# DassHydro-dev/smash

Hardware: AMD Instinct MI355X
Metric: cell-timesteps/s, forward+adjoint sweep (higher is better)
Workload: dtype f32

## Files before the change

### smash_amd/csrc/sx_kernels.h

```cpp
#pragma once

#include <hip/hip_runtime.h>

#include <climits>

#include "sx_ops.h"
#include "sx_tangent.h"
#include "sx_vic.h"

#define SX_BT 4
#define SX_VBLOCK 256

__device__ __forceinline__ void sx_lds_barrier() {
    __builtin_amdgcn_fence(__ATOMIC_RELEASE, "workgroup", "local");
    __builtin_amdgcn_s_barrier();
    __builtin_amdgcn_fence(__ATOMIC_ACQUIRE, "workgroup", "local");
}

__device__ __forceinline__ void sx_lds_wave_fence() {
    __builtin_amdgcn_fence(__ATOMIC_RELEASE, "workgroup", "local");
    __builtin_amdgcn_wave_barrier();
    __builtin_amdgcn_fence(__ATOMIC_ACQUIRE, "workgroup", "local");
}

typedef float sx_f4v __attribute__((ext_vector_type(4)));
__device__ __forceinline__ float4 sx_gload4(const float4* p) {
#if defined(__HIP_DEVICE_COMPILE__)
    const sx_f4v v = *(const __attribute__((address_space(1))) sx_f4v*)p;
    return make_float4(v.x, v.y, v.z, v.w);
#else
    return *p;
#endif
}
#ifndef SX_R_NT
#define SX_R_NT 0
#endif
__device__ __forceinline__ float4 sx_gload4s(const float4* p) {
#if defined(__HIP_DEVICE_COMPILE__)
    if (SX_R_NT & 1) {
        const sx_f4v v = __builtin_nontemporal_load((const __attribute__((address_space(1))) sx_f4v*)p);
        return make_float4(v.x, v.y, v.z, v.w);
    }
#endif
    return sx_gload4(p);
}
__device__ __forceinline__ void sx_gstore4s(float4* p, const float4& q) {
#if defined(__HIP_DEVICE_COMPILE__)
    if (SX_R_NT & 2) {
        sx_f4v v; v.x = q.x; v.y = q.y; v.z = q.z; v.w = q.w;
        __builtin_nontemporal_store(v, (__attribute__((address_space(1))) sx_f4v*)p);
        return;
    }
    {
        sx_f4v v; v.x = q.x; v.y = q.y; v.z = q.z; v.w = q.w;
        *(__attribute__((address_space(1))) sx_f4v*)p = v;
        return;
    }
#endif
    *p = q;
}
__device__ __forceinline__ void sx_gstore4(float4* p, const float4& q) {
#if defined(__HIP_DEVICE_COMPILE__)
    sx_f4v v; v.x = q.x; v.y = q.y; v.z = q.z; v.w = q.w;
    *(__attribute__((address_space(1))) sx_f4v*)p = v;
#else
    *p = q;
#endif
}
__device__ __forceinline__ float sx_gload1(const float* p) {
#if defined(__HIP_DEVICE_COMPILE__)
    return *(const __attribute__((address_space(1))) float*)p;
#else
    return *p;
#endif
}

__device__ __forceinline__ void sx_pin(float4& v) {
    asm volatile("" : "+v"(v.x), "+v"(v.y), "+v"(v.z), "+v"(v.w) : : "memory");
}

__device__ __forceinline__ void sx_pin1(float& v) { asm volatile("" : "+v"(v) : : "memory"); }
__device__ __forceinline__ void sx_pinu(unsigned& v) { asm volatile("" : "+v"(v) : : "memory"); }

typedef __attribute__((address_space(1))) int sx_gint;
#define SX_PROG_STALL(A) ((A).prog + (A).ngroups)
#define SX_PROG_TICKET(A) ((A).prog + (A).ngroups + 1)
#define SX_PROG_EXTRA 8
#ifndef SX_PK
#define SX_PK 16
#endif
#define SX_SPIN_LIMIT (1 << 22)
__device__ __forceinline__ void sx_wait_prog(const int* prog, int need, int& seen, int* stalled, int limit, int tag = -1) {
    if (seen >= need) return;
    int spins = 0;
    while (seen < need) {
        seen = __hip_atomic_load((const sx_gint*)prog, __ATOMIC_RELAXED, __HIP_MEMORY_SCOPE_AGENT);
        if (seen < need) {
            const bool out = ++spins > limit;
            if (out || (spins & 1023) == 0) {
                if (out) {
                    if (atomicCAS(stalled + 3, 0, tag + 2) == 0) { stalled[4] = (int)(prog - stalled); stalled[5] = need; stalled[6] = seen; }
                    __hip_atomic_store((sx_gint*)stalled, 1, __ATOMIC_RELAXED, __HIP_MEMORY_SCOPE_AGENT);
                }
                if (out || __hip_atomic_load((const sx_gint*)stalled, __ATOMIC_RELAXED, __HIP_MEMORY_SCOPE_AGENT)) { seen = 0x7fffffff; break; }
            }
            __builtin_amdgcn_s_sleep(32);
        }
    }
    __builtin_amdgcn_fence(__ATOMIC_ACQUIRE, "agent");
}
__device__ __forceinline__ void sx_publish(int* prog, int blocks) {
    __builtin_amdgcn_fence(__ATOMIC_RELEASE, "agent");
    __hip_atomic_store((sx_gint*)prog, blocks, __ATOMIC_RELAXED, __HIP_MEMORY_SCOPE_AGENT);
}

struct SxDeviceArrays {
    int n, npad, nt, Tc;
    int k0, k1;
    int nx;
    float dt, dx;
    const float* prcp; const float* pet;
    const unsigned short* prcp16; const float* petd; const float* pet_ratio;
    float prcp_c, prcp_gap; int hour0;
    float *ci, *cp, *cft, *cst, *exc, *lr;
    float* px[3]; float* px_b[3];
    float *rt_a, *rt_f, *rt_denf, *rt_denb;
    int* flwacc;
    float *hi, *hp, *hft, *hst, *hlr;
    float *ci_b, *cp_b, *cft_b, *cst_b, *exc_b, *lr_b, *hi_b, *hp_b, *hft_b, *hst_b, *hlr_b;
    float *qtT, *hrT;
    int hr_skew;
    float *qtdT, *xdT, *qgd;
    float* qdT;
    float *tape_hi, *tape_hp, *tape_hft, *tape_hst;
    float* ckpt_hi;
    float* xT;
    float* qsk; int cs0, ncs;
    float *qg, *qgb;
    int* cell_gauge;
    const int *g_slot_begin, *g_dmax;
    const int *s_cell, *s_stage, *s_sub, *s_wsub, *s_child, *s_ccount, *s_parent, *s_xout;
    const int *x_prod, *x_cons;
    int* prog;
    int ngroups;
    int spin_limit;
    int mute_group;
    long long* gtime;
};

struct SxStageTables {
    const int* wb_slot0; const int* wb_n; const int* wb_smin; const int* wb_spread;
    const int* fifo_g; const int* fifo_s;
};
#ifndef SX_STG_PF
#define SX_STG_PF 16
#endif
#ifndef SX_STG_WAVES
// ... 257 lines not shown
        sx_row_store4<SX_NT>(A.qtT + (size_t)tq * npad * 4, kb * 4u, q[0], q[1], q[2], q[3]);
    }
    A.hi[k] = husl1; A.hp[k] = husl2; A.hft[k] = hlsl;
}

#ifndef SX_VADJ_WAVES_VIC
#define SX_VADJ_WAVES_VIC 3
#endif
template <bool CF>
__global__ __launch_bounds__(SX_VBLOCK, SX_VADJ_WAVES_VIC) void sx_k_vert_adj_vic(SxDeviceArrays A, int t0, int T) {
    SX_LIBM_INIT();
    const int k = A.k0 + blockIdx.x * SX_VBLOCK + threadIdx.x;
    if (k >= A.k1) return;
    const size_t npad = (size_t)A.npad;
    const SxVicParams P = sx_vic_load(A, k);
    float cusl2_m4, cusl2_m5;
    sx_pow_m4_m5(P.cusl2, &cusl2_m4, &cusl2_m5);
    SxVicGrads G;
    G.b_b = A.ci_b[k]; G.cusl1_b = A.cp_b[k]; G.cusl2_b = A.cft_b[k]; G.clsl_b = A.cst_b[k]; G.ks_b = A.exc_b[k];
    G.ds_b = A.px_b[0][k]; G.dsm_b = A.px_b[1][k]; G.ws_b = A.px_b[2][k];
    G.husl1_b = A.hi_b[k]; G.husl2_b = A.hp_b[k]; G.hlsl_b = A.hft_b[k];
    const unsigned kb = (unsigned)k * 4u;
    SxForcing<CF> F(A, kb, t0 + T - 1);
    float n_h1 = 0.f, n_h2 = 0.f, n_hl = 0.f, n_q = 0.f;
    auto fetch = [&](int tt, bool first) {
        const size_t o = (size_t)tt * npad;
        F.template request<SX_VADJ_NT, true>(t0 + tt, first);
        n_h1 = sx_row_load<SX_VADJ_NT>(A.tape_hi + o, kb); n_h2 = sx_row_load<SX_VADJ_NT>(A.tape_hp + o, kb);
        n_hl = sx_row_load<SX_VADJ_NT>(A.tape_hft + o, kb);
        n_q = sx_row_load(A.qtT + (size_t)(tt >> 2) * npad * 4 + (tt & 3), kb * 4u);
    };
    if (T > 0) fetch(T - 1, true);
    for (int tt = T - 1; tt >= 0; --tt) {
        float h1 = n_h1, h2 = n_h2, hl = n_hl, q_b = n_q;
        F.hold();
        sx_pin1(h1); sx_pin1(h2); sx_pin1(hl); sx_pin1(q_b);
        if (tt > 0) fetch(tt - 1, false);
        sx_vic_step_b(P, cusl2_m4, cusl2_m5, F.prcp(), F.pet(), h1, h2, hl, q_b, G);
    }
    A.ci_b[k] = G.b_b; A.cp_b[k] = G.cusl1_b; A.cft_b[k] = G.cusl2_b; A.cst_b[k] = G.clsl_b; A.exc_b[k] = G.ks_b;
    A.px_b[0][k] = G.ds_b; A.px_b[1][k] = G.dsm_b; A.px_b[2][k] = G.ws_b;
    A.hi_b[k] = G.husl1_b; A.hp_b[k] = G.husl2_b; A.hft_b[k] = G.hlsl_b;
}

__global__ __launch_bounds__(SX_VBLOCK) void sx_k_vert_fwd_vic_d(SxDeviceArrays A, int t0, int T) {
    SX_LIBM_INIT();
    const int k = A.k0 + blockIdx.x * SX_VBLOCK + threadIdx.x;
    if (k >= A.k1) return;
    const size_t npad = (size_t)A.npad;
    const SxVicParams P = sx_vic_load(A, k);
    SxVicTan D;
    D.b_d = A.ci_b[k]; D.cusl1_d = A.cp_b[k]; D.cusl2_d = A.cft_b[k]; D.clsl_d = A.cst_b[k]; D.ks_d = A.exc_b[k];
    D.ds_d = A.px_b[0][k]; D.dsm_d = A.px_b[1][k]; D.ws_d = A.px_b[2][k];
    float cusl2_m4, cusl2_m5;
    sx_pow_m4_m5(P.cusl2, &cusl2_m4, &cusl2_m5);
    SxVD husl1 = sx_vd(A.hi[k], A.hi_b[k]), husl2 = sx_vd(A.hp[k], A.hp_b[k]), hlsl = sx_vd(A.hft[k], A.hft_b[k]);
    float* qt = A.qtT + (size_t)k * 4;
    float* qd = A.qtdT + (size_t)k * 4;
    for (int tt = 0; tt < T; ++tt) {
        float prcp, pet;
        sx_forcing_at(A, t0 + tt, (unsigned)k * 4u, prcp, pet);
        const SxVD r = sx_vic_step_d(P, D, cusl2_m4, cusl2_m5, prcp, pet, husl1, husl2, hlsl);
        const size_t o = (size_t)(tt >> 2) * npad * 4 + (tt & 3);
        qt[o] = r.v; qd[o] = r.d;
    }
    A.hi[k] = husl1.v; A.hi_b[k] = husl1.d; A.hp[k] = husl2.v; A.hp_b[k] = husl2.d; A.hft[k] = hlsl.v; A.hft_b[k] = hlsl.d;
}

template <int ST>
__global__ __launch_bounds__(SX_VBLOCK) void sx_k_vert_fwd_d(SxDeviceArrays A, int t0, int T) {
    SX_LIBM_INIT();
    const int k = A.k0 + blockIdx.x * SX_VBLOCK + threadIdx.x;
    if (k >= A.k1) return;
    const size_t npad = (size_t)A.npad;
    SxCellParams P;
    P.ci = (ST == 2 || ST == 3) ? A.ci[k] : 1.f;
    P.cp = A.cp[k];
    P.cft = A.cft[k];
    P.cst = (ST == 3) ? A.cst[k] : 1.f;
    P.exc = (ST != 4) ? A.exc[k] : 0.f;
    sx_cell_params_init(P);
    SxAdjParams Q;
    Q.cst_m5 = 1.f;
    sx_pow_m4_m5(P.cft, &P.cft_m4, &Q.cft_m5);
    P.cst_m4 = 1.f;
    if (ST == 3) sx_pow_m4_m5(P.cst, &P.cst_m4, &Q.cst_m5);
    Q.dcft2 = sx_mkdiv(P.cft * P.cft);
    Q.dcst2 = sx_mkdiv(P.cst * P.cst);
    Q.dcp2 = sx_mkdiv(P.cp * P.cp);
    SxTanParams D;
    D.ci_d = (ST == 2 || ST == 3) ? A.ci_b[k] : 0.f;
    D.cp_d = A.cp_b[k];
    D.cft_d = A.cft_b[k];
    D.cst_d = (ST == 3) ? A.cst_b[k] : 0.f;
    D.exc_d = (ST != 4) ? A.exc_b[k] : 0.f;
    SxDual hi = sx_mk(0.f, 0.f), hp, hft, hst = sx_mk(0.f, 0.f);
    if (ST == 2 || ST == 3) hi = sx_mk(A.hi[k], A.hi_b[k]);
    hp = sx_mk(A.hp[k], A.hp_b[k]);
    hft = sx_mk(A.hft[k], A.hft_b[k]);
    if (ST == 3) hst = sx_mk(A.hst[k], A.hst_b[k]);
    float4* qt4 = reinterpret_cast<float4*>(A.qtT) + k;
    float4* qd4 = reinterpret_cast<float4*>(A.qtdT) + k;
    for (int tq = 0; tq * 4 < T; ++tq) {
        float q[4] = {0.f, 0.f, 0.f, 0.f}, qd[4] = {0.f, 0.f, 0.f, 0.f};
#pragma unroll
        for (int i = 0; i < 4; ++i) {
            const int tt = tq * 4 + i;
            if (tt < T) {
                float prcp, pet;
                sx_forcing_at(A, t0 + tt, (unsigned)k * 4u, prcp, pet);
                const SxDual r = sx_vertical_step_d<ST>(P, Q, D, prcp, pet, hi, hp, hft, hst);
                q[i] = r.v; qd[i] = r.d;
            }
        }
        qt4[(size_t)tq * npad] = make_float4(q[0], q[1], q[2], q[3]);
        qd4[(size_t)tq * npad] = make_float4(qd[0], qd[1], qd[2], qd[3]);
    }
    if (ST == 2 || ST == 3) { A.hi[k] = hi.v; A.hi_b[k] = hi.d; }
    A.hp[k] = hp.v; A.hp_b[k] = hp.d;
    A.hft[k] = hft.v; A.hft_b[k] = hft.d;
    if (ST == 3) { A.hst[k] = hst.v; A.hst_b[k] = hst.d; }
}

#ifndef SX_MU
#define SX_MU 4
#endif
#ifndef SX_MU_F
#define SX_MU_F SX_MU
#endif
#ifndef SX_MU_A
#define SX_MU_A SX_MU
#endif
#ifndef SX_MAXGROUP
#define SX_MAXGROUP 512
#endif
#ifndef SX_R_PRIO
#define SX_R_PRIO 0
#endif
#ifndef SX_RLB_F
#define SX_RLB_F 1
#endif
#ifndef SX_RLB_A
#define SX_RLB_A 1
#endif

__device__ __forceinline__ int sx_next_ticket(const SxDeviceArrays& A) {
    __shared__ int s_ticket;
    __builtin_amdgcn_s_barrier();
    if (threadIdx.x == 0) s_ticket = __hip_atomic_fetch_add((sx_gint*)SX_PROG_TICKET(A), 1, __ATOMIC_RELAXED, __HIP_MEMORY_SCOPE_AGENT);
    __syncthreads();
    return s_ticket;
}

template <bool TAPE, bool CHAIN, int TMODE>
__device__ __forceinline__ void sx_route_fwd_group(const SxDeviceArrays& A, const int g, const int g0, const int gend, const int t0, const int T) {
    constexpr bool TAN = (TMODE == 2);
    constexpr int MU = SX_MU_F, PK = SX_PK * 4 / MU;
    constexpr bool DFORM = (TMODE == 1);
    extern __shared__ __attribute__((aligned(16))) float4 sx_lds[];
    const int sb = A.g_slot_begin[g], m = A.g_slot_begin[g + 1] - sb, dmax = A.g_dmax[g];
    const int j = threadIdx.x, M = blockDim.x;
    bool valid = j < m;
    const int nb = (T + SX_BT - 1) / SX_BT;
    if (A.gtime && j == 0) A.gtime[2 * g] = wall_clock64();

    int cell = -1, stage = 0, sub = 0, ccount = 0, xout = -1, xin = -1, gid = -1;
    unsigned ch01 = ~0u, ch23 = ~0u, ch45 = ~0u, ch67 = ~0u;
    float a = 0.f, f = 0.f, den = 1.f, hlr = 0.f, ad = 0.f;
    bool hasup = false;
    const int nsubw = __builtin_amdgcn_readfirstlane(m > 0 ? A.s_wsub[sb + min(j, m - 1)] : 1);
    if (valid && A.s_cell[sb + j] == INT_MIN) valid = false;
    if (valid) {
        const int c = A.s_cell[sb + j];
        stage = A.s_stage[sb + j];
        sub = A.s_sub[sb + j];
        if (c >= 0) {
            cell = c;
            const int4 cw = reinterpret_cast<const int4*>(A.s_child)[sb + j];
            ch01 = (unsigned)cw.x; ch23 = (unsigned)cw.y; ch45 = (unsigned)cw.z; ch67 = (unsigned)cw.w;
            ccount = A.s_ccount[sb + j]; xout = A.s_xout[sb + j];
            a = A.rt_a[c]; f = A.rt_f[c]; den = (TAN || DFORM) ? A.rt_denb[c] : A.rt_denf[c]; hlr = TAN ? A.hlr_b[c] : A.hlr[c];
            if (TAN) { const float lrv = A.lr[c]; ad = a * ((A.dt / (60.f * lrv)) * A.lr_b[c] / lrv); }
            hasup = A.flwacc[c] > 1;
            gid = A.cell_gauge[c];
        } else {
            xin = -1 - c;
        }
    }
    const float dt = A.dt, dx = A.dx;
    const SxDiv dden = sx_mkdiv(den), ddt = sx_mkdiv(dt);
    const int* wprog = nullptr;
    int seen = 0;
    if (CHAIN && xin >= 0) { const int pg = A.x_prod[xin]; if (pg >= g0 && pg < gend) wprog = A.prog + pg; }
    const bool staged = CHAIN && !TAN && A.qsk != nullptr && valid && !wprog;
    const float4* src = staged ? reinterpret_cast<const float4*>(A.qsk) + (size_t)stage * A.ncs + (sb + j - A.cs0)
                      : (cell >= 0) ? reinterpret_cast<const float4*>(TAN ? A.qtdT : A.qtT) + cell
                                    : reinterpret_cast<const float4*>(TAN ? A.xdT : A.xT) + (xin >= 0 ? xin : 0);
    const size_t sstride = staged ? (size_t)A.ncs : (cell >= 0) ? (size_t)A.npad : (size_t)A.nx;
    float4* x4 = reinterpret_cast<float4*>(TAN ? A.xdT : A.xT);
    float4* hr4 = reinterpret_cast<float4*>(A.hrT);
    const int hs = A.hr_skew ? stage : 0;
    float* gauge_out = TAN ? A.qgd : A.qg;
    const float4 zero4 = make_float4(0.f, 0.f, 0.f, 0.f);
    auto fetch = [&](int tb) -> float4 { return cell >= 0 ? sx_gload4s(src + (size_t)tb * sstride) : sx_gload4(src + (size_t)tb * sstride); };

    float4 nxt[MU], outq[MU], outh[MU], nhr[MU];
    if (CHAIN && wprog) sx_wait_prog(wprog, min(MU - stage, nb), seen, SX_PROG_STALL(A), A.spin_limit, g);
#pragma unroll
    for (int u = 0; u < MU; ++u) {
        const int tb = u - stage;
        nxt[u] = (valid && tb >= 0 && tb < nb) ? fetch(tb) : zero4;
        nhr[u] = (TAN && valid && cell >= 0 && tb >= 0 && tb < nb) ? sx_gload4(hr4 + (size_t)(tb + hs) * A.npad + cell) : zero4;
        outq[u] = zero4; outh[u] = zero4;
    }
    const int nsuper = nb + dmax;
    const int nmacro = (nsuper + MU - 1) / MU;
    for (int mw = 0; mw <= nmacro; ++mw) {
        float4 cur[MU], chr[MU];
#pragma unroll
        for (int u = 0; u < MU; ++u) { cur[u] = nxt[u]; sx_pin(cur[u]); if (TAN) { chr[u] = nhr[u]; sx_pin(chr[u]); } }
        if (CHAIN) asm volatile("s_waitcnt vmcnt(0)" ::: "memory");
        if (mw > 0 && cell >= 0) {
#pragma unroll
            for (int u = 0; u < MU; ++u) {
                const int tb = MU * (mw - 1) + u - stage;
                if (tb >= 0 && tb < nb) {
                    if (xout >= 0) x4[(size_t)tb * A.nx + xout] = outq[u];
                    if (TAPE) sx_gstore4s(hr4 + (size_t)(tb + hs) * A.npad + cell, outh[u]);
                    if (A.qdT) reinterpret_cast<float4*>(A.qdT)[(size_t)tb * A.npad + cell] = outq[u];
                    if (gid >= 0) {
                        const float qv[4] = {outq[u].x, outq[u].y, outq[u].z, outq[u].w};
#pragma unroll
                        for (int i = 0; i < SX_BT; ++i)
                            if (tb * SX_BT + i < T) gauge_out[(size_t)gid * A.nt + t0 + tb * SX_BT + i] = qv[i];
                    }
                }
            }
        }
        if (mw == nmacro) break;
        if (CHAIN && wprog) sx_wait_prog(wprog, min(MU * (mw + 2) - stage, nb), seen, SX_PROG_STALL(A), A.spin_limit, g);
#pragma unroll
        for (int u = 0; u < MU; ++u) {
            const int tb = MU * (mw + 1) + u - stage;
            nxt[u] = (valid && tb >= 0 && tb < nb) ? fetch(tb) : zero4;
            if (TAN) nhr[u] = (valid && cell >= 0 && tb >= 0 && tb < nb) ? sx_gload4(hr4 + (size_t)(tb + hs) * A.npad + cell) : zero4;
        }
#pragma unroll
        for (int u = 0; u < MU; ++u) {
            const int w = MU * mw + u;
            const int tb = w - stage;
            const bool act = valid && tb >= 0 && tb < nb;
            float4* pub = sx_lds + (size_t)(w & 1) * M;
            auto child_val = [&](unsigned e) -> float4 {
                const float4* row = sx_lds + (size_t)((w + 1 + (int)((e >> 15) & 1u)) & 1) * M;
                return row[min((int)(e & 0x7fffu), M - 1)];
            };
          auto sub_pass = [&](const int sl) {
            if (act && sub == sl) {
                const int tl = tb * SX_BT;
                if (cell >= 0) {
                    float s[SX_BT];
                    {
                        const float4 v0 = child_val(ch01 & 0xffffu), v1 = child_val(ch01 >> 16);
                        const bool h0 = ccount > 0, h1 = ccount > 1;
                        s[0] = (h0 ? v0.x : 0.f) + (h1 ? v1.x : 0.f); s[1] = (h0 ? v0.y : 0.f) + (h1 ? v1.y : 0.f);
                        s[2] = (h0 ? v0.z : 0.f) + (h1 ? v1.z : 0.f); s[3] = (h0 ? v0.w : 0.f) + (h1 ? v1.w : 0.f);
                    }
                    for (int c = 2; c < ccount; ++c) {
                        const unsigned wd = c < 4 ? ch23 : c < 6 ? ch45 : ch67;
                        const float4 v = child_val((wd >> ((c & 1) * 16)) & 0xffffu);
                        s[0] = s[0] + v.x; s[1] = s[1] + v.y; s[2] = s[2] + v.z; s[3] = s[3] + v.w;
                    }
                    const float qt[SX_BT] = {cur[u].x, cur[u].y, cur[u].z, cur[u].w};
                    float q[SX_BT], hr[SX_BT], qup[SX_BT], qro[SX_BT];
                    {
                        float nq[SX_BT], dq[SX_BT];
#pragma unroll
                        for (int i = 0; i < SX_BT; ++i) nq[i] = DFORM ? s[i] : s[i] * dt;
                        sx_div4(dq, nq, dden);
#pragma unroll
                        for (int i = 0; i < SX_BT; ++i) qup[i] = hasup ? (DFORM ? dt * dq[i] : dq[i]) : 0.f;
                    }
                    if (!TAN) {
#pragma unroll
                        for (int i = 0; i < SX_BT; ++i) {
                            const bool live = tl + i < T;
                            const float hr_imd = hlr + qup[i];
                            const float hnew = hr_imd * a;
                            qro[i] = hr_imd - hnew;
                            hr[i] = live ? hr_imd : 0.f;
                            hlr = live ? hnew : hlr;
                        }
                        float nq[SX_BT], dq[SX_BT];
#pragma unroll
                        for (int i = 0; i < SX_BT; ++i) nq[i] = DFORM ? qt[i] + f * qro[i] : (qt[i] + qro[i] * f) * dx * dx * 0.001f;
                        sx_div4(dq, nq, ddt);
#pragma unroll
                        for (int i = 0; i < SX_BT; ++i) {
                            const float v = DFORM ? (0.001f * (dx * dx)) * dq[i] : dq[i];
                            q[i] = (tl + i < T) ? v : 0.f;
                        }
                    } else {
                        const float hrv[SX_BT] = {chr[u].x, chr[u].y, chr[u].z, chr[u].w};
#pragma unroll
                        for (int i = 0; i < SX_BT; ++i) {
                            const bool live = tl + i < T;
                            const float hr_imd_d = hlr + qup[i];
                            const float hnew_d = a * hr_imd_d + hrv[i] * ad;
                            qro[i] = hr_imd_d - hnew_d;
                            hr[i] = 0.f;
                            hlr = live ? hnew_d : hlr;
                        }
#pragma unroll
                        for (int i = 0; i < SX_BT; ++i) {
                            const float v = sx_div((0.001f * (dx * dx)) * (qt[i] + f * qro[i]), ddt);
                            q[i] = (tl + i < T) ? v : 0.f;
                        }
                    }
                    const float4 q4 = make_float4(q[0], q[1], q[2], q[3]);
                    pub[j] = q4;
                    outq[u] = q4;
                    outh[u] = make_float4(hr[0], hr[1], hr[2], hr[3]);
                } else {
                    pub[j] = cur[u];
                }
            }
          };
            if (nsubw == 1) sub_pass(0);
            else for (int sl = 0; sl < nsubw; ++sl) { sub_pass(sl); if (sl + 1 < nsubw) sx_lds_wave_fence(); }
            sx_lds_barrier();
            if (CHAIN && u == 0 && j == 0 && mw % PK == 0) { const int done = min(MU * (mw - 1) - dmax, nb); if (done > 0 && g != A.mute_group) sx_publish(A.prog + g, done); }
        }
    }
    if (valid && cell >= 0) { if (TAN) A.hlr_b[cell] = hlr; else A.hlr[cell] = hlr; }
    if (A.gtime && j == 0) A.gtime[2 * g + 1] = wall_clock64();
    if (CHAIN) {
        asm volatile("s_waitcnt vmcnt(0)" ::: "memory");
        __builtin_amdgcn_s_barrier();
        if (j == 0 && g != A.mute_group) sx_publish(A.prog + g, nb);
    }
}

template <bool TAPE, bool CHAIN, int TMODE = 0>
__global__ __launch_bounds__(SX_MAXGROUP, SX_RLB_F) void sx_k_route_fwd(SxDeviceArrays A, int g0, int gend, int t0, int T) {
    if (SX_R_PRIO) __builtin_amdgcn_s_setprio(SX_R_PRIO);
    if (!CHAIN) { sx_route_fwd_group<TAPE, false, TMODE>(A, g0 + (int)blockIdx.x, g0, gend, t0, T); return; }
    for (;;) {
        const int ticket = sx_next_ticket(A);
        if (ticket >= gend - g0) break;
        sx_route_fwd_group<TAPE, CHAIN, TMODE>(A, g0 + ticket, g0, gend, t0, T);
    }
}

template <bool CHAIN>
__device__ __forceinline__ void sx_route_adj_group(const SxDeviceArrays& A, const int g, const int g0, const int gend, const int t0, const int T) {
    constexpr int MU = SX_MU_A, PK = SX_PK * 4 / MU;
    extern __shared__ __attribute__((aligned(16))) float4 sx_lds[];
    const int sb = A.g_slot_begin[g], m = A.g_slot_begin[g + 1] - sb, dmax = A.g_dmax[g];
    const int j = threadIdx.x, M = blockDim.x;
    bool valid = j < m;
    const int nb = (T + SX_BT - 1) / SX_BT;
    if (A.gtime && j == 0) A.gtime[2 * (A.ngroups + g)] = wall_clock64();

    int cell = -1, rstage = 0, sub = 0, par = -1, xout = -1, xin = -1, gid = -1;
    bool psame = false;
    float a = 0.f, f = 0.f, den = 1.f, lr = 1.f, hr_b = 0.f, lr_b = 0.f;
    bool hasup = false;
    const int nsubw = __builtin_amdgcn_readfirstlane(m > 0 ? A.s_wsub[sb + min(j, m - 1)] : 1);
    if (valid && A.s_cell[sb + j] == INT_MIN) valid = false;
    if (valid) {
        const int c = A.s_cell[sb + j];
        rstage = dmax - A.s_stage[sb + j];
        sub = A.s_sub[sb + j];
        par = A.s_parent[sb + j];
        if (par >= 0) { psame = (par & 0x40000000) != 0; par &= 0xffff; }
        if (c >= 0) {
            cell = c;
            xout = A.s_xout[sb + j];
            a = A.rt_a[c]; f = A.rt_f[c]; den = A.rt_denb[c]; lr = A.lr[c];
            hr_b = A.hlr_b[c]; lr_b = A.lr_b[c];
            hasup = A.flwacc[c] > 1;
            gid = A.cell_gauge[c];
        } else {
            xin = -1 - c;
        }
    }
    const float dt = A.dt, dx = A.dx;
    const SxDiv dden = sx_mkdiv(den), ddt = sx_mkdiv(dt), dlr = sx_mkdiv((lr * lr) * 60.f);
    float4* x4 = reinterpret_cast<float4*>(A.xT);
    const float4* hr4p = reinterpret_cast<const float4*>(A.hrT);
    const int hs = A.hr_skew ? dmax - rstage : 0;
    float4* qt4 = reinterpret_cast<float4*>(A.qtT);
    const float4 zero4 = make_float4(0.f, 0.f, 0.f, 0.f);
    const bool root_in = (cell >= 0 && par < 0 && xout >= 0);
    const bool staged = CHAIN && A.qsk != nullptr && valid && (cell >= 0 || (xin >= 0 && !(A.x_prod[xin] >= g0 && A.x_prod[xin] < gend)));
    float4* const dst = staged ? reinterpret_cast<float4*>(A.qsk) + (size_t)(dmax - rstage) * A.ncs + (sb + j - A.cs0)
                               : (cell >= 0) ? qt4 + cell : x4 + (xin >= 0 ? xin : 0);
    const size_t dstride = staged ? (size_t)A.ncs : (cell >= 0) ? (size_t)A.npad : (size_t)A.nx;

    const float* seedp = (gid >= 0) ? A.qgb + (size_t)gid * A.nt + t0 : nullptr;
    auto load_seed = [&](int tb) -> float4 {
        float4 v = make_float4(0.f, 0.f, 0.f, 0.f);
        if (gid >= 0) {
            const int tl = tb * SX_BT;
            if (tl + 0 < T) v.x = sx_gload1(seedp + tl + 0);
            if (tl + 1 < T) v.y = sx_gload1(seedp + tl + 1);
            if (tl + 2 < T) v.z = sx_gload1(seedp + tl + 2);
            if (tl + 3 < T) v.w = sx_gload1(seedp + tl + 3);
        }
        return v;
    };
    const int* wprog = nullptr;
    int seen = 0;
    if (CHAIN && root_in) { const int cg = A.x_cons[xout]; if (cg >= g0 && cg < gend) wprog = A.prog + cg; }
    auto fetch_in = [&](int tb) -> float4 { return sx_gload4(x4 + (size_t)tb * A.nx + xout); };
    float4 nhr[MU], nin[MU], nsd[MU], outq[MU];
    if (CHAIN && wprog) sx_wait_prog(wprog, min(MU - rstage, nb), seen, SX_PROG_STALL(A), A.spin_limit, g);
#pragma unroll
    for (int u = 0; u < MU; ++u) {
        const int tbr = u - rstage;
        const int tb = nb - 1 - tbr;
        const bool ok = valid && tbr >= 0 && tbr < nb;
        nhr[u] = (ok && cell >= 0) ? sx_gload4s(hr4p + (size_t)(tb + hs) * A.npad + cell) : zero4;
        nin[u] = (ok && root_in) ? fetch_in(tb) : zero4;
        nsd[u] = ok ? load_seed(tb) : zero4;
        outq[u] = zero4;
    }
    const int nsuper = nb + dmax;
    const int nmacro = (nsuper + MU - 1) / MU;
    for (int mw = 0; mw <= nmacro; ++mw) {
        float4 chr[MU], cin[MU], csd[MU];
#pragma unroll
        for (int u = 0; u < MU; ++u) {
            chr[u] = nhr[u]; cin[u] = nin[u]; csd[u] = nsd[u];
            sx_pin(chr[u]); sx_pin(cin[u]); sx_pin(csd[u]);
        }
        if (CHAIN) asm volatile("s_waitcnt vmcnt(0)" ::: "memory");
        if (mw > 0 && valid) {
#pragma unroll
            for (int u = 0; u < MU; ++u) {
                const int tbr = MU * (mw - 1) + u - rstage;
                if (tbr >= 0 && tbr < nb) {
                    const int tb = nb - 1 - tbr;
                    sx_gstore4(dst + (size_t)tb * dstride, outq[u]);
                }
            }
        }
        if (mw == nmacro) break;
        if (CHAIN && wprog) sx_wait_prog(wprog, min(MU * (mw + 2) - rstage, nb), seen, SX_PROG_STALL(A), A.spin_limit, g);
#pragma unroll
        for (int u = 0; u < MU; ++u) {
            const int tbr = MU * (mw + 1) + u - rstage;
            const int tb = nb - 1 - tbr;
            const bool ok = valid && tbr >= 0 && tbr < nb;
            nhr[u] = (ok && cell >= 0) ? sx_gload4s(hr4p + (size_t)(tb + hs) * A.npad + cell) : zero4;
            nin[u] = (ok && root_in) ? fetch_in(tb) : zero4;
            nsd[u] = ok ? load_seed(tb) : zero4;
        }
#pragma unroll
        for (int u = 0; u < MU; ++u) {
            const int w = MU * mw + u;
            const int tbr = w - rstage;
            const bool act = valid && tbr >= 0 && tbr < nb;
            float4* pub = sx_lds + (size_t)(w & 1) * M;
            const float4* prev = sx_lds + (size_t)((w + 1) & 1) * M;
          auto sub_pass = [&](const int sl) {
            if (act && sub == sl) {
                const int tb = nb - 1 - tbr;
                const int tl = tb * SX_BT;
                float4 in4 = cin[u];
                if (par >= 0) in4 = psame ? pub[par] : prev[par];
                if (cell >= 0) {
                    const float hrv[SX_BT] = {chr[u].x, chr[u].y, chr[u].z, chr[u].w};
                    const float inv[SX_BT] = {in4.x, in4.y, in4.z, in4.w};
                    const float sdv[SX_BT] = {csd[u].x, csd[u].y, csd[u].z, csd[u].w};
                    float pb[SX_BT], qtb[SX_BT];
                    float tmpb[SX_BT], qrb[SX_BT], himb[SX_BT], a1b[SX_BT];
                    float nq[SX_BT];
#pragma unroll
                    for (int i = SX_BT - 1; i >= 0; --i) {
                        float q_b = 0.f;
                        if (gid >= 0) q_b = q_b + sdv[i];
                        q_b = q_b + inv[i];
                        nq[i] = (dx * dx) * 0.001f * q_b;
                    }
                    sx_div4(tmpb, nq, ddt);
#pragma unroll
                    for (int i = SX_BT - 1; i >= 0; --i) qrb[i] = f * tmpb[i];
#pragma unroll
                    for (int i = SX_BT - 1; i >= 0; --i) {
                        const bool live = tl + i < T;
                        const float hb1 = hr_b - qrb[i];
                        himb[i] = qrb[i] + a * hb1;
                        a1b[i] = a * hrv[i] * hb1;
                        hr_b = live ? himb[i] : hr_b;
                    }
                    float na[SX_BT], nh[SX_BT], da[SX_BT], dh[SX_BT];
#pragma unroll
                    for (int i = 0; i < SX_BT; ++i) { na[i] = dt * a1b[i]; nh[i] = dt * himb[i]; }
                    sx_div4(da, na, dlr);
                    sx_div4(dh, nh, dden);
#pragma unroll
                    for (int i = SX_BT - 1; i >= 0; --i) {
                        const bool live = tl + i < T;
                        const float lnew = lr_b + da[i];
                        lr_b = live ? lnew : lr_b;
                        pb[i] = (live && hasup) ? dh[i] : 0.f;
                        qtb[i] = live ? tmpb[i] : 0.f;
                    }
                    pub[j] = make_float4(pb[0], pb[1], pb[2], pb[3]);
                    outq[u] = make_float4(qtb[0], qtb[1], qtb[2], qtb[3]);
                } else {
                    outq[u] = in4;
                }
            }
          };
            if (nsubw == 1) sub_pass(0);
            else for (int sl = nsubw - 1; sl >= 0; --sl) { sub_pass(sl); if (sl > 0) sx_lds_wave_fence(); }
            sx_lds_barrier();
            if (CHAIN && u == 0 && j == 0 && mw % PK == 0) { const int done = min(MU * (mw - 1) - dmax, nb); if (done > 0 && g != A.mute_group) sx_publish(A.prog + g, done); }
        }
    }
    if (valid && cell >= 0) { A.hlr_b[cell] = hr_b; A.lr_b[cell] = lr_b; }
    if (A.gtime && j == 0) A.gtime[2 * (A.ngroups + g) + 1] = wall_clock64();
    if (CHAIN) {
        asm volatile("s_waitcnt vmcnt(0)" ::: "memory");
        __builtin_amdgcn_s_barrier();
        if (j == 0 && g != A.mute_group) sx_publish(A.prog + g, nb);
    }
}

template <bool CHAIN>
__global__ __launch_bounds__(SX_MAXGROUP, SX_RLB_A) void sx_k_route_adj(SxDeviceArrays A, int g0, int gend, int t0, int T) {
    if (SX_R_PRIO) __builtin_amdgcn_s_setprio(SX_R_PRIO);
    if (!CHAIN) { sx_route_adj_group<false>(A, g0 + (int)blockIdx.x, g0, gend, t0, T); return; }
    for (;;) {
        const int ticket = sx_next_ticket(A);
        if (ticket >= gend - g0) break;
        sx_route_adj_group<CHAIN>(A, gend - 1 - ticket, g0, gend, t0, T);
    }
}

#ifndef SX_VADJ_WAVES
#define SX_VADJ_WAVES 5
#endif
template <int ST, bool CF>
#ifndef SX_VADJ_WAVES_GRC
#if SX_EXACT_LIBM
#define SX_VADJ_WAVES_GRC 1
#else
#define SX_VADJ_WAVES_GRC 5
#endif
#endif
__global__ __launch_bounds__(SX_VBLOCK, (ST == 2 && CF) ? SX_VADJ_WAVES : (ST == 3 && CF) ? SX_VADJ_WAVES_GRC : 1)
void sx_k_vert_adj(SxDeviceArrays A, int t0, int T) {
    SX_LIBM_INIT();
    const int k = A.k0 + blockIdx.x * SX_VBLOCK + threadIdx.x;
    if (k >= A.k1) return;
    const size_t npad = (size_t)A.npad;
    SxCellParams P;
    P.ci = (ST == 2 || ST == 3) ? A.ci[k] : 1.f;
    P.cp = A.cp[k];
    P.cft = A.cft[k];
    P.cst = (ST == 3) ? A.cst[k] : 1.f;
    P.exc = (ST != 4) ? A.exc[k] : 0.f;
    sx_cell_params_init(P);
    SxAdjParams Q;
    Q.cst_m5 = 1.f;
    sx_pow_m4_m5(P.cft, &P.cft_m4, &Q.cft_m5);
    P.cst_m4 = 1.f;
    if (ST == 3) sx_pow_m4_m5(P.cst, &P.cst_m4, &Q.cst_m5);
    Q.dcft2 = sx_mkdiv(P.cft * P.cft);
    Q.dcst2 = sx_mkdiv(P.cst * P.cst);
    Q.dcp2 = sx_mkdiv(P.cp * P.cp);
    SxCellGrads G;
    G.ci_b = (ST == 2 || ST == 3) ? A.ci_b[k] : 0.f;
    G.cp_b = A.cp_b[k];
    G.cft_b = A.cft_b[k];
    G.cst_b = (ST == 3) ? A.cst_b[k] : 0.f;
    G.exc_b = (ST != 4) ? A.exc_b[k] : 0.f;
    G.hi_b = (ST == 2 || ST == 3) ? A.hi_b[k] : 0.f;
    G.hp_b = A.hp_b[k];
    G.hft_b = A.hft_b[k];
    G.hst_b = (ST == 3) ? A.hst_b[k] : 0.f;
    const unsigned kb = (unsigned)k * 4u;
    SxForcing<CF> F(A, kb, t0 + T - 1);
    float n_hi = 0.f, n_hp = 0.f, n_hft = 0.f, n_hst = 0.f, n_q = 0.f;
    const bool hi_taped = (ST == 2 || ST == 3) && A.tape_hi != nullptr;
    const size_t olast = (size_t)(T > 0 ? T - 1 : 0) * npad;
    const float* r_hi = hi_taped ? A.tape_hi + olast : nullptr;
    const float* r_hp = A.tape_hp + olast;
    const float* r_hft = A.tape_hft + olast;
    const float* r_hst = (ST == 3) ? A.tape_hst + olast : nullptr;
    auto fetch = [&](int tt, bool first) {
        F.template request<SX_VADJ_NT, true>(t0 + tt, first);
        if (hi_taped) { n_hi = sx_row_load<SX_VADJ_NT>(r_hi, kb); r_hi -= npad; }
        n_hp = sx_row_load<SX_VADJ_NT>(r_hp, kb); n_hft = sx_row_load<SX_VADJ_NT>(r_hft, kb);
        r_hp -= npad; r_hft -= npad;
        if (ST == 3) { n_hst = sx_row_load<SX_VADJ_NT>(r_hst, kb); r_hst -= npad; }
        n_q = sx_row_load(A.qtT + (size_t)(tt >> 2) * npad * 4 + (tt & 3), kb * 4u);
    };
    __shared__ float s_hi[(ST == 2 || ST == 3) ? SX_HIK : 1][SX_VBLOCK];
    if (T > 0) fetch(T - 1, true);
    for (int tb = (T - 1) / SX_HIK; tb >= 0; --tb) {
        const int tt0 = tb * SX_HIK, len = min(SX_HIK, T - tt0);
        if ((ST == 2 || ST == 3) && !hi_taped) {
            float fp[SX_HIK], fe[SX_HIK];
#pragma unroll
            for (int j = 0; j < SX_HIK; ++j) sx_forcing_at(A, t0 + tt0 + (j < len ? j : 0), kb, fp[j], fe[j]);
            float h = sx_row_load(A.ckpt_hi + (size_t)tb * npad, kb);
#pragma unroll
            for (int j = 0; j < SX_HIK; ++j) {
                s_hi[j][threadIdx.x] = h;
                if (j < len && fp[j] >= 0.f && fe[j] >= 0.f) { float pn, ei; sx_interception(fp[j], fe[j], P.ci, P.dci, h, pn, ei); }
            }
        }
        for (int tt = tt0 + len - 1; tt >= tt0; --tt) {
            float hit = n_hi, hp = n_hp, hft = n_hft, hst = n_hst, q = n_q;
            F.hold();
            sx_pin1(hp); sx_pin1(hft); sx_pin1(q);
            if (ST == 2 || ST == 3) sx_pin1(hit);
            if (ST == 3) sx_pin1(hst);
            if (tt > 0) fetch(tt - 1, false);
            const float prcp = F.prcp(), pet = F.pet();
            const float hi = (ST == 2 || ST == 3) ? (hi_taped ? hit : s_hi[tt - tt0][threadIdx.x]) : 0.f;
            const bool still = SX_STILL && sx_wave_all(sx_is_still<ST>(prcp, pet, hi, hp));
            sx_vertical_step_b<ST>(P, Q, prcp, pet, hi, hp, hft, hst, q, G, still);
        }
    }
    if (ST == 2 || ST == 3) { A.ci_b[k] = G.ci_b; A.hi_b[k] = G.hi_b; }
    A.cp_b[k] = G.cp_b;
    A.cft_b[k] = G.cft_b;
    if (ST == 3) { A.cst_b[k] = G.cst_b; A.hst_b[k] = G.hst_b; }
    if (ST != 4) A.exc_b[k] = G.exc_b;
    A.hp_b[k] = G.hp_b;
    A.hft_b[k] = G.hft_b;
}
```

Measured before the change: 54.49 billion.

## Specialise routing kernels on time tail and strength-reduce per-step address math

Adds a TAIL template parameter so routing kernels drop the per-timestep bounds checks when T is a multiple of the block size. Replaces per-iteration 64-bit index multiplies with running address pointers for the source, destination and hr tape streams. In the adjoint it skips inflow and seed loads for waves where no lane needs them, and uses a single-subpass specialisation that simplifies the LDS parent read. The goal is fewer VALU/SALU instructions and lower register pressure in the latency-bound routing sweep, at the cost of doubling kernel instantiations and making the address arithmetic harder to follow.

```diff
diff --git a/smash_amd/csrc/sx_kernels.h b/smash_amd/csrc/sx_kernels.h
--- a/smash_amd/csrc/sx_kernels.h
+++ b/smash_amd/csrc/sx_kernels.h
@@ -3,6 +3,7 @@
 #include <hip/hip_runtime.h>
 
 #include <climits>
+#include <type_traits>
 
 #include "sx_ops.h"
 #include "sx_tangent.h"
@@ -566,7 +567,12 @@
     return s_ticket;
 }
 
-template <bool TAPE, bool CHAIN, int TMODE>
+typedef unsigned long long sx_addr;
+__device__ __forceinline__ sx_addr sx_row_addr(const void* base, ptrdiff_t elems) { return (sx_addr)base + (sx_addr)elems * sizeof(float4); }
+__device__ __forceinline__ sx_addr sx_rows(int s, ptrdiff_t row) { return (sx_addr)((ptrdiff_t)s * row) * sizeof(float4); }
+__device__ __forceinline__ float4* sx_at(sx_addr a) { return reinterpret_cast<float4*>(a); }
+
+template <bool TAPE, bool CHAIN, int TMODE, bool TAIL>
 __device__ __forceinline__ void sx_route_fwd_group(const SxDeviceArrays& A, const int g, const int g0, const int gend, const int t0, const int T) {
     constexpr bool TAN = (TMODE == 2);
     constexpr int MU = SX_MU_F, PK = SX_PK * 4 / MU;
@@ -610,21 +616,27 @@
     const float4* src = staged ? reinterpret_cast<const float4*>(A.qsk) + (size_t)stage * A.ncs + (sb + j - A.cs0)
                       : (cell >= 0) ? reinterpret_cast<const float4*>(TAN ? A.qtdT : A.qtT) + cell
                                     : reinterpret_cast<const float4*>(TAN ? A.xdT : A.xT) + (xin >= 0 ? xin : 0);
-    const size_t sstride = staged ? (size_t)A.ncs : (cell >= 0) ? (size_t)A.npad : (size_t)A.nx;
+    const int sstride = staged ? A.ncs : (cell >= 0) ? A.npad : A.nx;
     float4* x4 = reinterpret_cast<float4*>(TAN ? A.xdT : A.xT);
     float4* hr4 = reinterpret_cast<float4*>(A.hrT);
-    const int hs = A.hr_skew ? stage : 0;
     float* gauge_out = TAN ? A.qgd : A.qg;
     const float4 zero4 = make_float4(0.f, 0.f, 0.f, 0.f);
-    auto fetch = [&](int tb) -> float4 { return cell >= 0 ? sx_gload4s(src + (size_t)tb * sstride) : sx_gload4(src + (size_t)tb * sstride); };
+    sx_addr scur = sx_row_addr(src, -(ptrdiff_t)stage * (ptrdiff_t)sstride);
+    auto fetch = [&]() -> float4 { return cell >= 0 ? sx_gload4s(sx_at(scur)) : sx_gload4(sx_at(scur)); };
+    const ptrdiff_t crow = (ptrdiff_t)A.npad;
+    auto hr_at = [&](int s, int tb) -> float4* {
+        if (A.hr_skew) return reinterpret_cast<float4*>(reinterpret_cast<char*>(hr4 + (ptrdiff_t)s * crow) + (unsigned)cell * (unsigned)sizeof(float4));
+        return hr4 + (size_t)tb * A.npad + cell;
+    };
 
     float4 nxt[MU], outq[MU], outh[MU], nhr[MU];
     if (CHAIN && wprog) sx_wait_prog(wprog, min(MU - stage, nb), seen, SX_PROG_STALL(A), A.spin_limit, g);
 #pragma unroll
     for (int u = 0; u < MU; ++u) {
         const int tb = u - stage;
-        nxt[u] = (valid && tb >= 0 && tb < nb) ? fetch(tb) : zero4;
-        nhr[u] = (TAN && valid && cell >= 0 && tb >= 0 && tb < nb) ? sx_gload4(hr4 + (size_t)(tb + hs) * A.npad + cell) : zero4;
+        nxt[u] = (valid && tb >= 0 && tb < nb) ? fetch() : zero4;
+        scur += (sx_addr)sstride * sizeof(float4);
+        nhr[u] = (TAN && valid && cell >= 0 && tb >= 0 && tb < nb) ? sx_gload4(hr_at(u, tb)) : zero4;
         outq[u] = zero4; outh[u] = zero4;
     }
     const int nsuper = nb + dmax;
@@ -637,16 +649,17 @@
         if (mw > 0 && cell >= 0) {
 #pragma unroll
             for (int u = 0; u < MU; ++u) {
-                const int tb = MU * (mw - 1) + u - stage;
+                const int s = MU * (mw - 1) + u;
+                const int tb = s - stage;
                 if (tb >= 0 && tb < nb) {
                     if (xout >= 0) x4[(size_t)tb * A.nx + xout] = outq[u];
-                    if (TAPE) sx_gstore4s(hr4 + (size_t)(tb + hs) * A.npad + cell, outh[u]);
+                    if (TAPE) sx_gstore4s(hr_at(s, tb), outh[u]);
                     if (A.qdT) reinterpret_cast<float4*>(A.qdT)[(size_t)tb * A.npad + cell] = outq[u];
                     if (gid >= 0) {
                         const float qv[4] = {outq[u].x, outq[u].y, outq[u].z, outq[u].w};
 #pragma unroll
                         for (int i = 0; i < SX_BT; ++i)
-                            if (tb * SX_BT + i < T) gauge_out[(size_t)gid * A.nt + t0 + tb * SX_BT + i] = qv[i];
+                            if (!TAIL || tb * SX_BT + i < T) gauge_out[(size_t)gid * A.nt + t0 + tb * SX_BT + i] = qv[i];
                     }
                 }
             }
@@ -655,9 +668,11 @@
         if (CHAIN && wprog) sx_wait_prog(wprog, min(MU * (mw + 2) - stage, nb), seen, SX_PROG_STALL(A), A.spin_limit, g);
 #pragma unroll
         for (int u = 0; u < MU; ++u) {
-            const int tb = MU * (mw + 1) + u - stage;
-            nxt[u] = (valid && tb >= 0 && tb < nb) ? fetch(tb) : zero4;
-            if (TAN) nhr[u] = (valid && cell >= 0 && tb >= 0 && tb < nb) ? sx_gload4(hr4 + (size_t)(tb + hs) * A.npad + cell) : zero4;
+            const int s = MU * (mw + 1) + u;
+            const int tb = s - stage;
+            nxt[u] = (valid && tb >= 0 && tb < nb) ? fetch() : zero4;
+            scur += (sx_addr)sstride * sizeof(float4);
+            if (TAN) nhr[u] = (valid && cell >= 0 && tb >= 0 && tb < nb) ? sx_gload4(hr_at(s, tb)) : zero4;
         }
 #pragma unroll
         for (int u = 0; u < MU; ++u) {
@@ -698,7 +713,7 @@
                     if (!TAN) {
 #pragma unroll
                         for (int i = 0; i < SX_BT; ++i) {
-                            const bool live = tl + i < T;
+                            const bool live = !TAIL || tl + i < T;
                             const float hr_imd = hlr + qup[i];
                             const float hnew = hr_imd * a;
                             qro[i] = hr_imd - hnew;
@@ -712,13 +727,13 @@
 #pragma unroll
                         for (int i = 0; i < SX_BT; ++i) {
                             const float v = DFORM ? (0.001f * (dx * dx)) * dq[i] : dq[i];
-                            q[i] = (tl + i < T) ? v : 0.f;
+                            q[i] = (!TAIL || tl + i < T) ? v : 0.f;
                         }
                     } else {
                         const float hrv[SX_BT] = {chr[u].x, chr[u].y, chr[u].z, chr[u].w};
 #pragma unroll
                         for (int i = 0; i < SX_BT; ++i) {
-                            const bool live = tl + i < T;
+                            const bool live = !TAIL || tl + i < T;
                             const float hr_imd_d = hlr + qup[i];
                             const float hnew_d = a * hr_imd_d + hrv[i] * ad;
                             qro[i] = hr_imd_d - hnew_d;
@@ -728,7 +743,7 @@
 #pragma unroll
                         for (int i = 0; i < SX_BT; ++i) {
                             const float v = sx_div((0.001f * (dx * dx)) * (qt[i] + f * qro[i]), ddt);
-                            q[i] = (tl + i < T) ? v : 0.f;
+                            q[i] = (!TAIL || tl + i < T) ? v : 0.f;
                         }
                     }
                     const float4 q4 = make_float4(q[0], q[1], q[2], q[3]);
@@ -758,15 +773,21 @@
 template <bool TAPE, bool CHAIN, int TMODE = 0>
 __global__ __launch_bounds__(SX_MAXGROUP, SX_RLB_F) void sx_k_route_fwd(SxDeviceArrays A, int g0, int gend, int t0, int T) {
     if (SX_R_PRIO) __builtin_amdgcn_s_setprio(SX_R_PRIO);
-    if (!CHAIN) { sx_route_fwd_group<TAPE, false, TMODE>(A, g0 + (int)blockIdx.x, g0, gend, t0, T); return; }
+    const bool tail = T % SX_BT != 0;
+    if (!CHAIN) {
+        if (tail) sx_route_fwd_group<TAPE, false, TMODE, true>(A, g0 + (int)blockIdx.x, g0, gend, t0, T);
+        else sx_route_fwd_group<TAPE, false, TMODE, false>(A, g0 + (int)blockIdx.x, g0, gend, t0, T);
+        return;
+    }
     for (;;) {
         const int ticket = sx_next_ticket(A);
         if (ticket >= gend - g0) break;
-        sx_route_fwd_group<TAPE, CHAIN, TMODE>(A, g0 + ticket, g0, gend, t0, T);
-    }
-}
-
-template <bool CHAIN>
+        if (tail) sx_route_fwd_group<TAPE, CHAIN, TMODE, true>(A, g0 + ticket, g0, gend, t0, T);
+        else sx_route_fwd_group<TAPE, CHAIN, TMODE, false>(A, g0 + ticket, g0, gend, t0, T);
+    }
+}
+
+template <bool CHAIN, bool TAIL>
 __device__ __forceinline__ void sx_route_adj_group(const SxDeviceArrays& A, const int g, const int g0, const int gend, const int t0, const int T) {
     constexpr int MU = SX_MU_A, PK = SX_PK * 4 / MU;
     extern __shared__ __attribute__((aligned(16))) float4 sx_lds[];
@@ -810,24 +831,28 @@
     const bool staged = CHAIN && A.qsk != nullptr && valid && (cell >= 0 || (xin >= 0 && !(A.x_prod[xin] >= g0 && A.x_prod[xin] < gend)));
     float4* const dst = staged ? reinterpret_cast<float4*>(A.qsk) + (size_t)(dmax - rstage) * A.ncs + (sb + j - A.cs0)
                                : (cell >= 0) ? qt4 + cell : x4 + (xin >= 0 ? xin : 0);
-    const size_t dstride = staged ? (size_t)A.ncs : (cell >= 0) ? (size_t)A.npad : (size_t)A.nx;
+    const int dstride = staged ? A.ncs : (cell >= 0) ? A.npad : A.nx;
 
     const float* seedp = (gid >= 0) ? A.qgb + (size_t)gid * A.nt + t0 : nullptr;
     auto load_seed = [&](int tb) -> float4 {
         float4 v = make_float4(0.f, 0.f, 0.f, 0.f);
         if (gid >= 0) {
             const int tl = tb * SX_BT;
-            if (tl + 0 < T) v.x = sx_gload1(seedp + tl + 0);
-            if (tl + 1 < T) v.y = sx_gload1(seedp + tl + 1);
-            if (tl + 2 < T) v.z = sx_gload1(seedp + tl + 2);
-            if (tl + 3 < T) v.w = sx_gload1(seedp + tl + 3);
+            if (!TAIL || tl + 0 < T) v.x = sx_gload1(seedp + tl + 0);
+            if (!TAIL || tl + 1 < T) v.y = sx_gload1(seedp + tl + 1);
+            if (!TAIL || tl + 2 < T) v.z = sx_gload1(seedp + tl + 2);
+            if (!TAIL || tl + 3 < T) v.w = sx_gload1(seedp + tl + 3);
         }
         return v;
     };
+    const bool wave_seed = __ballot(gid >= 0) != 0ull, wave_in = __ballot(root_in) != 0ull;
     const int* wprog = nullptr;
     int seen = 0;
     if (CHAIN && root_in) { const int cg = A.x_cons[xout]; if (cg >= g0 && cg < gend) wprog = A.prog + cg; }
+    const ptrdiff_t crow = (ptrdiff_t)A.npad;
+    const sx_addr hrl = sx_row_addr(hr4p, (ptrdiff_t)(nb - 1 + rstage + hs) * crow + (cell >= 0 ? cell : 0));
     auto fetch_in = [&](int tb) -> float4 { return sx_gload4(x4 + (size_t)tb * A.nx + xout); };
+    sx_addr dcur = sx_row_addr(dst, (ptrdiff_t)(nb - 1 + rstage) * (ptrdiff_t)dstride);
     float4 nhr[MU], nin[MU], nsd[MU], outq[MU];
     if (CHAIN && wprog) sx_wait_prog(wprog, min(MU - rstage, nb), seen, SX_PROG_STALL(A), A.spin_limit, g);
 #pragma unroll
@@ -835,9 +860,10 @@
         const int tbr = u - rstage;
         const int tb = nb - 1 - tbr;
         const bool ok = valid && tbr >= 0 && tbr < nb;
-        nhr[u] = (ok && cell >= 0) ? sx_gload4s(hr4p + (size_t)(tb + hs) * A.npad + cell) : zero4;
-        nin[u] = (ok && root_in) ? fetch_in(tb) : zero4;
-        nsd[u] = ok ? load_seed(tb) : zero4;
+        nhr[u] = (ok && cell >= 0) ? sx_gload4s(sx_at(hrl - sx_rows(u, crow))) : zero4;
+        nin[u] = zero4; nsd[u] = zero4;
+        if (wave_in) nin[u] = (ok && root_in) ? fetch_in(tb) : zero4;
+        if (wave_seed) nsd[u] = ok ? load_seed(tb) : zero4;
         outq[u] = zero4;
     }
     const int nsuper = nb + dmax;
@@ -845,31 +871,35 @@
     for (int mw = 0; mw <= nmacro; ++mw) {
         float4 chr[MU], cin[MU], csd[MU];
 #pragma unroll
-        for (int u = 0; u < MU; ++u) {
-            chr[u] = nhr[u]; cin[u] = nin[u]; csd[u] = nsd[u];
-            sx_pin(chr[u]); sx_pin(cin[u]); sx_pin(csd[u]);
+        for (int u = 0; u < MU; ++u) { chr[u] = nhr[u]; sx_pin(chr[u]); cin[u] = zero4; csd[u] = zero4; }
+        if (wave_in) {
+#pragma unroll
+            for (int u = 0; u < MU; ++u) { cin[u] = nin[u]; sx_pin(cin[u]); }
+        }
+        if (wave_seed) {
+#pragma unroll
+            for (int u = 0; u < MU; ++u) { csd[u] = nsd[u]; sx_pin(csd[u]); }
         }
         if (CHAIN) asm volatile("s_waitcnt vmcnt(0)" ::: "memory");
         if (mw > 0 && valid) {
 #pragma unroll
             for (int u = 0; u < MU; ++u) {
                 const int tbr = MU * (mw - 1) + u - rstage;
-                if (tbr >= 0 && tbr < nb) {
-                    const int tb = nb - 1 - tbr;
-                    sx_gstore4(dst + (size_t)tb * dstride, outq[u]);
-                }
+                if (tbr >= 0 && tbr < nb) sx_gstore4(sx_at(dcur), outq[u]);
+                dcur -= (sx_addr)dstride * sizeof(float4);
             }
         }
         if (mw == nmacro) break;
         if (CHAIN && wprog) sx_wait_prog(wprog, min(MU * (mw + 2) - rstage, nb), seen, SX_PROG_STALL(A), A.spin_limit, g);
 #pragma unroll
         for (int u = 0; u < MU; ++u) {
-            const int tbr = MU * (mw + 1) + u - rstage;
+            const int s = MU * (mw + 1) + u;
+            const int tbr = s - rstage;
             const int tb = nb - 1 - tbr;
             const bool ok = valid && tbr >= 0 && tbr < nb;
-            nhr[u] = (ok && cell >= 0) ? sx_gload4s(hr4p + (size_t)(tb + hs) * A.npad + cell) : zero4;
-            nin[u] = (ok && root_in) ? fetch_in(tb) : zero4;
-            nsd[u] = ok ? load_seed(tb) : zero4;
+            nhr[u] = (ok && cell >= 0) ? sx_gload4s(sx_at(hrl - sx_rows(s, crow))) : zero4;
+            if (wave_in) nin[u] = (ok && root_in) ? fetch_in(tb) : zero4;
+            if (wave_seed) nsd[u] = ok ? load_seed(tb) : zero4;
         }
 #pragma unroll
         for (int u = 0; u < MU; ++u) {
@@ -878,12 +908,13 @@
             const bool act = valid && tbr >= 0 && tbr < nb;
             float4* pub = sx_lds + (size_t)(w & 1) * M;
             const float4* prev = sx_lds + (size_t)((w + 1) & 1) * M;
-          auto sub_pass = [&](const int sl) {
-            if (act && sub == sl) {
+          auto sub_pass = [&](const int sl, auto one) {
+            constexpr bool ONE = decltype(one)::value;
+            if (act && (ONE || sub == sl)) {
                 const int tb = nb - 1 - tbr;
                 const int tl = tb * SX_BT;
-                float4 in4 = cin[u];
-                if (par >= 0) in4 = psame ? pub[par] : prev[par];
+                const float4 lv = ((!ONE && psame) ? pub : prev)[par >= 0 ? par : j];
+                const float4 in4 = par >= 0 ? lv : cin[u];
                 if (cell >= 0) {
                     const float hrv[SX_BT] = {chr[u].x, chr[u].y, chr[u].z, chr[u].w};
                     const float inv[SX_BT] = {in4.x, in4.y, in4.z, in4.w};
@@ -903,7 +934,7 @@
                     for (int i = SX_BT - 1; i >= 0; --i) qrb[i] = f * tmpb[i];
 #pragma unroll
                     for (int i = SX_BT - 1; i >= 0; --i) {
-                        const bool live = tl + i < T;
+                        const bool live = !TAIL || tl + i < T;
                         const float hb1 = hr_b - qrb[i];
                         himb[i] = qrb[i] + a * hb1;
                         a1b[i] = a * hrv[i] * hb1;
@@ -916,7 +947,7 @@
                     sx_div4(dh, nh, dden);
 #pragma unroll
                     for (int i = SX_BT - 1; i >= 0; --i) {
-                        const bool live = tl + i < T;
+                        const bool live = !TAIL || tl + i < T;
                         const float lnew = lr_b + da[i];
                         lr_b = live ? lnew : lr_b;
                         pb[i] = (live && hasup) ? dh[i] : 0.f;
@@ -929,8 +960,8 @@
                 }
             }
           };
-            if (nsubw == 1) sub_pass(0);
-            else for (int sl = nsubw - 1; sl >= 0; --sl) { sub_pass(sl); if (sl > 0) sx_lds_wave_fence(); }
+            if (nsubw == 1) sub_pass(0, std::true_type());
+            else for (int sl = nsubw - 1; sl >= 0; --sl) { sub_pass(sl, std::false_type()); if (sl > 0) sx_lds_wave_fence(); }
             sx_lds_barrier();
             if (CHAIN && u == 0 && j == 0 && mw % PK == 0) { const int done = min(MU * (mw - 1) - dmax, nb); if (done > 0 && g != A.mute_group) sx_publish(A.prog + g, done); }
         }
@@ -947,11 +978,17 @@
 template <bool CHAIN>
 __global__ __launch_bounds__(SX_MAXGROUP, SX_RLB_A) void sx_k_route_adj(SxDeviceArrays A, int g0, int gend, int t0, int T) {
     if (SX_R_PRIO) __builtin_amdgcn_s_setprio(SX_R_PRIO);
-    if (!CHAIN) { sx_route_adj_group<false>(A, g0 + (int)blockIdx.x, g0, gend, t0, T); return; }
+    const bool tail = T % SX_BT != 0;
+    if (!CHAIN) {
+        if (tail) sx_route_adj_group<false, true>(A, g0 + (int)blockIdx.x, g0, gend, t0, T);
+        else sx_route_adj_group<false, false>(A, g0 + (int)blockIdx.x, g0, gend, t0, T);
+        return;
+    }
     for (;;) {
         const int ticket = sx_next_ticket(A);
         if (ticket >= gend - g0) break;
-        sx_route_adj_group<CHAIN>(A, gend - 1 - ticket, g0, gend, t0, T);
+        if (tail) sx_route_adj_group<CHAIN, true>(A, gend - 1 - ticket, g0, gend, t0, T);
+        else sx_route_adj_group<CHAIN, false>(A, gend - 1 - ticket, g0, gend, t0, T);
     }
 }
 
```

Result: faster. 55.43 billion (median of 6 runs) (+1.7%).
